# HybridRobotics/ilqr-iterative-tasks

Measured on AMD Instinct MI355X. Metric: batched iLQR iterations/s (n=6,m=2,N=20), higher is better.
Workload: dtype f64

## Files before the change

ilqr_iterative_tasks_amd/csrc/i2lqr_abi.hip:

```cpp
#include <hip/hip_runtime.h>
#include <dlfcn.h>
#include <rccl/rccl.h>

#include <atomic>
#include <cmath>
#include <cstdarg>
#include <cstdio>
#include <cstdlib>
#include <cstring>
#include <mutex>
#include <new>
#include <unordered_set>

#include "../../include/i2lqr.h"
#include "i2lqr_devcfg.hpp"
#include "i2lqr_geometry.hpp"
#include "i2lqr_group.h"
#include "i2lqr_lane.hpp"
#include "i2lqr_select.hpp"
#include "i2lqr_wave.hpp"

#include "i2lqr_lane12.h"

#define I2LQR_DRY_RUN_LANE 1
// ... 233 lines not shown
}

struct i2lqr_handle {
  i2lqr_config cfg;
  int lanes;
  size_t lds_bytes;
  int device;
  void* ws;
  int64_t ws_bytes;
  int64_t compact_min_batch;
  int opt_defer, opt_reroll, opt_lds_steps, opt_merge, opt_ckpt, opt_stagger;
  int wave_tail;
  int opt_pair;
  int opt_two_x;
  int opt_chunk_step;
  int opt_fuse;
  int opt_final_round;
  int opt_first_chunk;
  int opt_fstep;
  int opt_group;
  int opt_spec;
  int opt_group_ws;
  int opt_group_overlap;
  struct Epilogue {
    const int32_t* qfun;
    int outer_iter, max_relax_iter;
    void* cost_it;
    void* part;
    int64_t* best_idx;
    void* best_cost;
    bool fused;
  };
  static constexpr unsigned kTickets = 16;
  unsigned* ticket;
  std::atomic<unsigned> ticket_next;
  hipEvent_t ev_ready, ev_side_done;
  bool side_pending;
  DeviceGeometry geo;
};

namespace {
thread_local i2lqr_handle::Epilogue* t_epi = nullptr;
}

namespace {

// ... 142 lines not shown
        a.best_idx = t_epi->best_idx;
        a.best_cost = (T*)t_epi->best_cost;
      }
      t_epi->fused = true;
    }
    switch (fk) {
      case K_INVALID:
        return fail(I2LQR_ERR_UNSUPPORTED, "%s", why);
      case K_SPEC:
      case K_SPEC16:
        if constexpr (m == 2 && n + m <= 8) {
          HIP_TRY(group_spec_iterate<T>(h->cfg, a, s, fk == K_SPEC16 ? 16 : 8));
          return I2LQR_OK;
        }
        break;
      case K_GROUP:
        if constexpr (m == 2 && n + m <= 8) {
          HIP_TRY(group_iterate<T>(h->cfg, a, s));
          return I2LQR_OK;
        }
        break;
      case K_GROUP16:
        if constexpr (m == 2 && n + m <= 8) {
          HIP_TRY(group16_iterate<T>(h->cfg, a, s, h->opt_group_overlap != 0));
          return I2LQR_OK;
        }
        break;
      case K_GROUP_WS:
        if constexpr (m == 2 && n + m <= 8) {
          HIP_TRY(group_iterate_ws<T>(h->cfg, a, h->ws, s));
          return I2LQR_OK;
        }
        break;
      case K_QUAD:
        if constexpr (n + m == 16) {
          HIP_TRY(quad_iterate<T>(h->cfg, a, h->ws, s));
          return I2LQR_OK;
        }
        break;
      case K_WAVE:
        break;
    }
    const size_t lds_f = fstep_lds_bytes(h->cfg.N);
    const int64_t waves_per_cu = (grid(B) + h->geo.cus - 1) / h->geo.cus;
    const bool fstep = kHasFstep && lds_f <= h->geo.default_dyn_lds &&
                       (h->opt_fstep >= 0 ? h->opt_fstep != 0
                                          : waves_per_cu * lds_f <= h->geo.lds_per_cu - 10 * 1024);
// ... 812 lines not shown
#ifdef I2LQR_DRY_RUN
  const bool dry_run = dry::on();
#else
  constexpr bool dry_run = false;
#endif
  if (!dry_run && (hipGetDeviceCount(&ndev) != hipSuccess || ndev <= 0))
    return fail(I2LQR_ERR_NODEVICE, "no HIP device visible (this library has no CPU path)");
  i2lqr_handle* h = new (std::nothrow) i2lqr_handle;
  if (!h) return fail(I2LQR_ERR_LAUNCH, "out of host memory");
  h->cfg = *cfg;
  h->geo = device_geometry();
  if (h->geo.wave != 64) {
    const int w = h->geo.wave;
    delete h;
    return fail(I2LQR_ERR_UNSUPPORTED, "the kernels are built for 64-lane wavefronts (gfx950), this "
                "device reports %d", w);
  }
  h->ws = nullptr;
  h->ws_bytes = 0;
  h->compact_min_batch = -1;
  h->opt_defer = h->opt_reroll = h->opt_lds_steps = h->opt_fstep = h->opt_group = -1;
  h->opt_merge = h->opt_ckpt = h->opt_spec = h->opt_stagger = h->opt_group_ws = -1;
  h->opt_group_overlap = -1;
  h->wave_tail = -1;
  h->opt_first_chunk = -1;
  h->opt_fuse = -1;
  h->opt_final_round = -1;
  h->opt_chunk_step = -1;
  h->opt_pair = -1;
  h->opt_two_x = -1;
  h->ticket = nullptr;
  h->ticket_next.store(0);
  h->ev_ready = h->ev_side_done = nullptr;
  h->side_pending = false;
  constexpr size_t kTicketBytes = i2lqr_handle::kTickets * sizeof(unsigned);
  if (dry_run) {
#ifdef I2LQR_DRY_RUN
    static unsigned fake_tickets[i2lqr_handle::kTickets];
    h->device = 0;
    h->ticket = fake_tickets;
    dry::allow(fake_tickets, sizeof(fake_tickets));
#endif
  } else if (hipGetDevice(&h->device) != hipSuccess ||
      hipMalloc((void**)&h->ticket, kTicketBytes) != hipSuccess ||
      hipMemset(h->ticket, 0, kTicketBytes) != hipSuccess) {
    if (h->ticket) (void)hipFree(h->ticket);
// ... 152 lines not shown
}

int i2lqr_set_option(i2lqr_handle* h, const char* name, int64_t value) {
  if (!h || !name) return fail(I2LQR_ERR_INVALID, "null handle or option name");
  if (value < -1 || value > 0x7fffffff) return fail(I2LQR_ERR_INVALID, "option value out of range");
  const int v = (int)value;
  if (!strcmp(name, "defer_states")) h->opt_defer = v < 0 ? -1 : (v != 0);
  else if (!strcmp(name, "reroll_nominal")) h->opt_reroll = v < 0 ? -1 : (v != 0);
  else if (!strcmp(name, "lds_gain_steps")) h->opt_lds_steps = v;
  else if (!strcmp(name, "merge_inputs")) h->opt_merge = v < 0 ? -1 : (v != 0);
  else if (!strcmp(name, "checkpoint_states")) h->opt_ckpt = v < 0 ? -1 : (v != 0);
  else if (!strcmp(name, "stagger")) h->opt_stagger = v;
  else if (!strcmp(name, "per_step_jacobians")) h->opt_fstep = v < 0 ? -1 : (v != 0);
  else if (!strcmp(name, "wave_tail")) h->wave_tail = v < 0 ? -1 : (v > 65536 ? 65536 : v);
  else if (!strcmp(name, "first_chunk")) h->opt_first_chunk = v < 1 ? -1 : (v > 1024 ? 1024 : v);
  else if (!strcmp(name, "helper_wavefront")) h->opt_pair = v < 0 ? -1 : (v != 0);
  else if (!strcmp(name, "state_buffers")) h->opt_two_x = v < 0 ? -1 : (v != 0);
  else if (!strcmp(name, "chunk_step")) h->opt_chunk_step = v < 1 ? -1 : (v > 1024 ? 1024 : v);
  else if (!strcmp(name, "fused_compaction")) h->opt_fuse = v < 0 ? -1 : (v != 0);
  else if (!strcmp(name, "final_round")) h->opt_final_round = v < 0 ? -1 : (v > 20 ? 20 : v);
  else if (!strcmp(name, "speculate")) h->opt_spec = v < 0 ? -1 : (v != 0);
  else if (!strcmp(name, "group_workspace")) h->opt_group_ws = v < 0 ? -1 : (v != 0);
  else if (!strcmp(name, "group_overlap")) h->opt_group_overlap = v < 0 ? -1 : (v != 0);
  else if (!strcmp(name, "debug_self_test")) {
#ifdef I2LQR_DEBUG
    unsigned long long* w = i2lqr::debug_trap_word();
    double* buf = nullptr;
    HIP_TRY(hipMalloc((void**)&buf, 8 * sizeof(double)));
    hipLaunchKernelGGL(k_debug_self_test, dim3(1), dim3(64), 0, (hipStream_t)0, buf, w);
    const int rc = debug_check(I2LQR_OK, nullptr);
    (void)hipFree(buf);
    return rc;
#else
    return fail(I2LQR_ERR_UNSUPPORTED, "\"debug_self_test\" exists in the index-checked debug build "
                "only (make -C ilqr_iterative_tasks_amd/csrc debug)");
#endif
  }
  else if (!strcmp(name, "group_lanes")) {
    if (v != -1 && v != 8 && v != 16 && v != 64)
      return fail(I2LQR_ERR_INVALID, "\"group_lanes\" is 8, 16, 64 or -1");
    h->opt_group = v;
  }
  else return fail(I2LQR_ERR_INVALID, "unknown option '%s'", name);
  return I2LQR_OK;
}

// ... 588 lines not shown
```

ilqr_iterative_tasks_amd/csrc/i2lqr_group.h:

```cpp
#pragma once
#include <hip/hip_runtime.h>

#include "../../include/i2lqr.h"
#include "i2lqr_wave.hpp"

namespace i2lqr {

bool group_supported(const i2lqr_config& cfg);
template <class T> hipError_t group_iterate(const i2lqr_config& cfg, const IterArgs<T>& a,
                                            hipStream_t stream);

constexpr int64_t kGroup16Batch = 4096;
bool group16_supported(const i2lqr_config& cfg);
template <class T> hipError_t group16_iterate(const i2lqr_config& cfg, const IterArgs<T>& a,
                                              hipStream_t stream, bool overlap = true);

constexpr int64_t kGroupWsBatch = 4096;
constexpr int64_t kGroupWsTop = 8192;
constexpr int64_t kGroupWsTopF32 = 7168;
inline int64_t group_ws_top(const i2lqr_config& cfg) {
  return cfg.dtype == I2LQR_F64 ? kGroupWsTop : kGroupWsTopF32;
}
int64_t group_workspace_bytes(const i2lqr_config& cfg, int64_t B);
template <class T> hipError_t group_iterate_ws(const i2lqr_config& cfg, const IterArgs<T>& a,
                                               void* ws, hipStream_t stream);

bool group_spec_supported(const i2lqr_config& cfg, int lanes);
template <class T> hipError_t group_spec_iterate(const i2lqr_config& cfg, const IterArgs<T>& a,
                                                 hipStream_t stream, int lanes);
bool group_spec_chain_supported(const i2lqr_config& cfg, int64_t chains);
template <class T> hipError_t group_spec_chain(const i2lqr_config& cfg, const IterArgs<T>& a,
                                               hipStream_t stream);
bool group_spec_tail_supported(const i2lqr_config& cfg);
template <class T> hipError_t group_spec_tail(const i2lqr_config& cfg, const IterArgs<T>& a,
                                              hipStream_t stream);

bool quad_supported(const i2lqr_config& cfg);
int64_t quad_workspace_bytes(const i2lqr_config& cfg, int64_t B);
// ... 5 lines not shown
```

ilqr_iterative_tasks_amd/csrc/i2lqr_group.hip:

```cpp
#include "i2lqr_group.h"

#include "i2lqr_devcfg.hpp"
#include "i2lqr_geometry.hpp"
#include "i2lqr_group.hpp"
#include "i2lqr_dryrun.hpp"

namespace i2lqr {

namespace {

template <class T, class Sys, int G = kGroup> size_t group_lds_bytes(int N) {
  return (size_t)GLayout<Sys, G>(N).wave_words() * sizeof(T);
}

template <auto Kernel> hipError_t raise_lds_limit(size_t lds) {
  if (lds <= device_geometry().default_dyn_lds) return hipSuccess;
  constexpr int kMaxDev = 64;
  static thread_local int raised_for[kMaxDev] = {};
  int dev = 0;
  hipError_t e = hipGetDevice(&dev);
  if (e != hipSuccess) return e;
  if (dev < 0 || dev >= kMaxDev || raised_for[dev] < (int)lds) {
    e = hipFuncSetAttribute((const void*)Kernel, hipFuncAttributeMaxDynamicSharedMemorySize,
                            (int)lds);
    if (e != hipSuccess) return e;
    if (dev >= 0 && dev < kMaxDev) raised_for[dev] = (int)lds;
  }
  return hipSuccess;
}

template <class T, class Sys, int H, int G = kGroup>
hipError_t launch_h(const i2lqr_config& cfg, const IterArgs<T>& a, hipStream_t s) {
  const auto c = make_dev_cfg<T, Sys::n, Sys::m>(cfg);
  const size_t lds = group_lds_bytes<T, Sys, G>(cfg.N);
  if (hipError_t e = raise_lds_limit<k_group_iterate<T, Sys, H, false, G>>(lds); e != hipSuccess)
    return e;
  constexpr int PW = 64 / G;
  const unsigned grid = (unsigned)((a.B + PW - 1) / PW);
  hipLaunchKernelGGL((k_group_iterate<T, Sys, H, false, G>), dim3(grid), dim3(64 * H), lds, s, c, a,
                     (T*)nullptr);
  return hipGetLastError();
}
template <class T, class Sys>
hipError_t launch16(const i2lqr_config& cfg, const IterArgs<T>& a, hipStream_t s, bool overlap) {
  const int64_t cus = device_geometry().cus;
#ifndef I2LQR_STAMPS
  if (overlap && (a.B + 3) / 4 <= cus) return launch_h<T, Sys, 3, 16>(cfg, a, s);
  if ((a.B + 3) / 4 <= 2 * cus) return launch_h<T, Sys, 2, 16>(cfg, a, s);
#endif
  return launch_h<T, Sys, 1, 16>(cfg, a, s);
}
template <class T, class Sys>
hipError_t launch_ws(const i2lqr_config& cfg, const IterArgs<T>& a, void* ws, hipStream_t s) {
  const auto c = make_dev_cfg<T, Sys::n, Sys::m>(cfg);
  const size_t lds = (size_t)GLayout<Sys>(cfg.N, true).wave_words() * sizeof(T);
  if (hipError_t e = raise_lds_limit<k_group_iterate<T, Sys, 1, true>>(lds); e != hipSuccess) return e;
  const unsigned grid = (unsigned)((a.B + kGroupsPerWave - 1) / kGroupsPerWave);
  hipLaunchKernelGGL((k_group_iterate<T, Sys, 1, true>), dim3(grid), dim3(64), lds, s, c, a, (T*)ws);
  return hipGetLastError();
}

template <class T, class Sys>
hipError_t launch(const i2lqr_config& cfg, const IterArgs<T>& a, hipStream_t s) {
  const int64_t cus = device_geometry().cus;
#ifndef I2LQR_STAMPS
  if ((a.B + kGroupsPerWave - 1) / kGroupsPerWave <= cus) return launch_h<T, Sys, 3>(cfg, a, s);
#endif
  return launch_h<T, Sys, 1>(cfg, a, s);
}

constexpr int kSpecWideBatch = 512;

// ... 76 lines not shown
  if (chains > geo.scaled(kSpecWideBatch)) return false;
  const size_t lds = visit_bicycle(cfg, [&](auto t, auto sys) {
    return spec_lds_bytes<decltype(t), decltype(sys), 3, 16>(cfg.N);
  });
  return lds <= geo.max_dyn_lds;
}
template <class T>
hipError_t group_spec_chain(const i2lqr_config& cfg, const IterArgs<T>& a, hipStream_t s) {
  return visit_bicycle<T>(cfg, [&](auto, auto sys) {
    return launch_spec_chain<T, decltype(sys)>(cfg, a, s);
  });
}
template <class T>
hipError_t group_spec_iterate(const i2lqr_config& cfg, const IterArgs<T>& a, hipStream_t s, int lanes) {
  return launch_spec_any<T, false>(cfg, a, s, lanes);
}
template <class T>
hipError_t group_spec_tail(const i2lqr_config& cfg, const IterArgs<T>& a, hipStream_t s) {
  return launch_spec_any<T, true>(cfg, a, s, group_spec_tail_lanes(cfg));
}

bool group16_supported(const i2lqr_config& cfg) { return group_lds_fits<16>(cfg); }
template <class T>
hipError_t group16_iterate(const i2lqr_config& cfg, const IterArgs<T>& a, hipStream_t s, bool overlap) {
  return visit_bicycle<T>(cfg, [&](auto, auto sys) {
    return launch16<T, decltype(sys)>(cfg, a, s, overlap);
  });
}

bool group_supported(const i2lqr_config& cfg) { return group_lds_fits<kGroup>(cfg); }

int64_t group_workspace_bytes(const i2lqr_config& cfg, int64_t B) {
  if (!group_supported(cfg) || B <= 0) return 0;
  const int64_t probs = (B + kGroupsPerWave - 1) / kGroupsPerWave * kGroupsPerWave;
  const int64_t words = visit_bicycle<double>(cfg, [&](auto, auto sys) {
    return GLayout<decltype(sys)>(cfg.N, true).ws_words();
  });
  const size_t lds = visit_bicycle(cfg, [&](auto t, auto sys) {
    return (size_t)GLayout<decltype(sys)>(cfg.N, true).wave_words() * sizeof(t);
  });
  if (lds > device_geometry().max_dyn_lds) return 0;
  return probs * words * (cfg.dtype == I2LQR_F64 ? 8 : 4);
}
template <class T>
hipError_t group_iterate_ws(const i2lqr_config& cfg, const IterArgs<T>& a, void* ws, hipStream_t s) {
  return visit_bicycle<T>(cfg, [&](auto, auto sys) {
    return launch_ws<T, decltype(sys)>(cfg, a, ws, s);
  });
}

template <class T>
hipError_t group_iterate(const i2lqr_config& cfg, const IterArgs<T>& a, hipStream_t s) {
  return visit_bicycle<T>(cfg, [&](auto, auto sys) { return launch<T, decltype(sys)>(cfg, a, s); });
}

#define I2LQR_GROUP_LAUNCHERS(T)                                                                    \
  template hipError_t group_iterate<T>(const i2lqr_config&, const IterArgs<T>&, hipStream_t);       \
  template hipError_t group16_iterate<T>(const i2lqr_config&, const IterArgs<T>&, hipStream_t, bool); \
  template hipError_t group_iterate_ws<T>(const i2lqr_config&, const IterArgs<T>&, void*,           \
                                          hipStream_t);                                             \
  template hipError_t group_spec_iterate<T>(const i2lqr_config&, const IterArgs<T>&, hipStream_t,   \
                                            int);                                                   \
  template hipError_t group_spec_chain<T>(const i2lqr_config&, const IterArgs<T>&, hipStream_t);    \
  template hipError_t group_spec_tail<T>(const i2lqr_config&, const IterArgs<T>&, hipStream_t);
I2LQR_GROUP_LAUNCHERS(double)
I2LQR_GROUP_LAUNCHERS(float)

}
```

ilqr_iterative_tasks_amd/csrc/i2lqr_group.hpp:

```cpp
#pragma once
#include <hip/hip_runtime.h>
#include <stdint.h>

#include "i2lqr_systems.hpp"
#include "i2lqr_wave.hpp"

namespace i2lqr {

constexpr int kGroup = 8;
constexpr int kGroupsPerWave = 64 / kGroup;

template <class Sys> struct GroupPattern {
  static constexpr int n = Sys::n, m = Sys::m, W = n + m, NV = Sys::NVAR;
  static constexpr int dt_row(int b) {
    for (int i = 2; i < n; i++)
      if (i != b && Sys::pat(i, b) == 2) return i;
    return -1;
  }
  static constexpr bool column_ok(int b) {
    int extra = 0;
    for (int i = 0; i < n; i++) {
      const int code = Sys::pat(i, b);
      if (i < 2) {
        if (code == 2) return false;
// ... 61 lines not shown
template <int L, class T, int R>
__device__ __forceinline__ void bcast_fmac(T (&a)[R], const T (&s)[R], T c) {
#pragma unroll
  for (int r = 0; r < R; r++) bcast_fmac1<L>(a[r], s[r], c);
}
template <int L> __device__ __forceinline__ double bcast_mov(double v) {
  long long x = __builtin_bit_cast(long long, v);
  x = __builtin_amdgcn_mov_dpp(x, 0x150 + L, 0xf, 0xf, false);
  return __builtin_bit_cast(double, x);
}
template <int L> __device__ __forceinline__ float bcast_mov(float v) {
  int x = __builtin_bit_cast(int, v);
  x = __builtin_amdgcn_mov_dpp(x, 0x150 + L, 0xf, 0xf, false);
  return __builtin_bit_cast(float, x);
}
template <class T, int R> __device__ __forceinline__ void dpp_ready(T (&v)[R]) {
  if constexpr (R == 8)
    asm("s_nop 1" : "+v"(v[0]), "+v"(v[1]), "+v"(v[2]), "+v"(v[3]), "+v"(v[4]), "+v"(v[5]), "+v"(v[6]), "+v"(v[7]));
  else if constexpr (R == 6)
    asm("s_nop 1" : "+v"(v[0]), "+v"(v[1]), "+v"(v[2]), "+v"(v[3]), "+v"(v[4]), "+v"(v[5]));
  else static_assert(R == 6 || R == 8, "dpp_ready: n + m of the bicycles");
}

template <class T, class Sys, bool WS = false, int G = kGroup> struct GroupWorker {
  static constexpr int n = Sys::n, m = Sys::m, W = n + m, NV = Sys::NVAR, NT = Sys::NTRIG;
  static constexpr int NA = n + 1;
  using Cfg = DevCfg<T, n, m>;
  using GL = GLayout<Sys, G>;
  static_assert(G == kGroup || G == 16, "eight lanes per problem, or one 16-lane DPP row");
  static_assert(G == kGroup || !WS, "the workspace form is built for eight lanes per problem");
  using GP = GroupPattern<Sys>;
  static_assert(GP::ok(), "plant does not have the column structure this kernel is written for");
  const Cfg& c;
  const GL L;
  const Slice<T> S;
  const T* const Qt;
  const int g;
  const int N;
  int oR, oKk;
  T* T1c;
  int rho;
  T* Wp = nullptr;

  int off_c0, off_c1;
  int off_l0, off_l1;
  int off_lu[m];
  T own, cdt;
  int rsrc;
#ifdef I2LQR_STAMPS
  mutable unsigned long long st_acc[8] = {0, 0, 0, 0, 0, 0, 0, 0}, st_t0 = 0, st_t1 = 0;
#endif

  __device__ GroupWorker(const Cfg& c_, T* smem, int lane)
      : GroupWorker(c_, smem + (lane / G) * GL(c_.N, WS).total,
                    smem + GL(c_.N, WS).qt_base(), lane % G,
                    GL(c_.N, WS).total) {
    const int p = lane / G;
    if constexpr (G == kGroup) T1c = smem + L.t1_base() + p * GL::kT1Stride;
    rho = (p >> 1) & 1;
  }
  __device__ __forceinline__ T* rec(int t) const {
    if constexpr (WS) return Wp + L.ws_rec() + t * GL::RW;
    else return S + oR + t * GL::RW;
  }
  __device__ __forceinline__ T* gain(int t) const {
    if constexpr (WS) return Wp + L.ws_gain() + t * (m * GL::KW);
    else return S + oKk + t * (m * GL::KW);
  }
  __device__ __forceinline__ T* gain_x(int t) const {
    if constexpr (WS) return S + oKk;
    else return S + oKk + t * (m * GL::KW);
  }
  __device__ __forceinline__ void ws_publish() const {
    if constexpr (WS) {
      __builtin_amdgcn_fence(__ATOMIC_RELEASE, "workgroup");
      __builtin_amdgcn_s_waitcnt(0);
      wave_sync();
      __builtin_amdgcn_fence(__ATOMIC_ACQUIRE, "workgroup");
    }
  }
  __device__ __forceinline__ int t1_word(int col, int row) const {
    return (row >> 1) * (2 * kGroup) + ((col + rho) & (kGroup - 1)) * 2 + (row & 1);
  }

  __device__ GroupWorker(const Cfg& c_, T* slice, const T* qt, int g_, int slice_words)
      : c(c_), L(c_.N, WS), S(make_slice(slice, slice_words, c_.trap, TAG_GROUP_LDS)), Qt(qt),
        g(g_), N(c_.N) {
    oR = L.R; oKk = L.Kk;
    T1c = nullptr;
    rho = 0;
    off_c0 = GL::R_ZERO; off_c1 = GL::R_ZERO; off_l0 = GL::R_ZERO; off_l1 = GL::R_ZERO;
#pragma unroll
    for (int a = 0; a < m; a++) off_lu[a] = GL::R_ZERO;
    own = T(0); cdt = T(0); rsrc = 0;
    static_for_i<0, W>([&](auto b_) {
      constexpr int b = decltype(b_)::value;
      if (g == b && b < n) {
        constexpr int c0 = Sys::pat(0, b), c1 = Sys::pat(1, b);
        off_c0 = c0 == 0 ? GL::R_ZERO : (c0 == 1 ? GL::R_ONE : GL::R_JV + (c0 - 3));
        off_c1 = c1 == 0 ? GL::R_ZERO : (c1 == 1 ? GL::R_ONE : GL::R_JV + (c1 - 3));
        own = (b >= 2) ? T(1) : T(0);
        constexpr int r = GP::dt_row(b);
        cdt = r >= 0 ? c.dt : T(0);
        rsrc = r >= 0 ? r : 0;
        if (b < 2) {
          off_l0 = GL::R_OB + 2 + b;
          off_l1 = GL::R_OB + 3 + b;
        }
      }
    });
// ... 25 lines not shown
    }
    return acc;
  }

  template <int i, int a> __device__ __forceinline__ void f_acc(T& acc, bool& first, T v,
                                                                const T (&jv)[NV]) const {
    constexpr int code = Sys::pat(i, a);
    if constexpr (code == 0) {
      return;
    } else if constexpr (code == 1) {
      acc = first ? v : acc + v;
      first = false;
    } else {
      const T f = code == 2 ? c.dt : jv[code >= 3 ? code - 3 : 0];
      acc = first ? f * v : t_fma(f, v, acc);
      first = false;
    }
  }

  __device__ __forceinline__ T rollout(int XUo, int TRo, const T (&xT)[n]) const {
    T x[n], u[m], xn[n], tr[NT];
#pragma unroll
    for (int i = 0; i < n; i++) x[i] = S[XUo + i];
    for (int t = 0; t < N; t++) {
#pragma unroll
      for (int a = 0; a < m; a++) u[a] = clip(S[XUo + t * W + n + a], -c.u_max[a], c.u_max[a]);
#pragma unroll
      for (int a = 0; a < m; a++) S[XUo + t * W + n + a] = u[a];
      Sys::trig(x, tr);
#pragma unroll
      for (int q = 0; q < NT; q++) S[TRo + t * NT + q] = tr[q];
      Sys::step_tr(c, x, u, tr, xn);
#pragma unroll
      for (int i = 0; i < n; i++) S[XUo + (t + 1) * W + i] = xn[i];
#pragma unroll
      for (int i = 0; i < n; i++) x[i] = xn[i];
    }
    Sys::trig(x, tr);
#pragma unroll
    for (int q = 0; q < NT; q++) S[TRo + N * NT + q] = tr[q];
    const T cost = terminal_cost(x, xT);
    wave_sync();
    return cost;
  }

  __device__ __forceinline__ void prep(int XUo, int TRo, const T (&ob)[6], T pa, T pb, int first,
// ... 243 lines not shown
      for (int r = 0; r < n; r++) vx += (T(2) * Qt[i * n + r]) * dx[r];
      const T vxx = T(2) * Qt[i * n + gq];
      vb[i] = (g == n) ? vx : (g < n ? vxx : T(0));
    }
  }
  template <bool GENERAL>
  __device__ __forceinline__ bool backward_row_from(const T (&vb)[n], T lamb, bool commit) const {
    static_assert(GL::KW > n + 1, "the padding word of a gain row takes the stores of idle lanes");
    bool bad = false;
    T va[n];
    {
      const T* Rn = rec(N);
#pragma unroll
      for (int i = 0; i < n; i++) va[i] = vb[i];
      va[0] += Rn[off_l0];
      va[1] += Rn[off_l1];
    }
    const int gcol = (commit && g <= n) ? g : GL::KW - 1;
    T cdr[n];
#pragma unroll
    for (int r = 0; r < n; r++) cdr[r] = (rsrc == r) ? cdt : T(0);
    struct Rec { T jv[NV], luu[m], c0, c1, l0, l1, lrow[m]; };
    Rec ra, rb;
    auto load_record = [&](int t, Rec& r) __attribute__((always_inline)) {
      const T* R = rec(t);
#pragma unroll
      for (int q = 0; q < NV; q++) r.jv[q] = R[GL::R_JV + q];
#pragma unroll
      for (int a = 0; a < m; a++) r.luu[a] = R[GL::R_LUU + a];
      r.c0 = R[off_c0];
      r.c1 = R[off_c1];
      r.l0 = R[off_l0];
      r.l1 = R[off_l1];
#pragma unroll
      for (int a = 0; a < m; a++) r.lrow[a] = R[off_lu[a]];
    };
    auto f_entry = [&](auto k_, auto b_, const T (&jv)[NV]) __attribute__((always_inline)) {
      constexpr int code = Sys::pat(decltype(k_)::value, n + decltype(b_)::value);
      if constexpr (code == 1) return T(1);
      else if constexpr (code == 2) return c.dt;
      else return jv[code >= 3 ? code - 3 : 0];
    };
    load_record(N - 1, ra);
    auto step = [&](const int t, Rec& rc, Rec& rn) __attribute__((always_inline)) {
      const T (&jv)[NV] = rc.jv;
      T t1[W];
      static_for_i<0, W>([&](auto a_) {
        constexpr int a = decltype(a_)::value;
        T acc = T(0);
        bool first = true;
        static_for_i<0, n>([&](auto i_) {
          constexpr int i = decltype(i_)::value;
          f_acc<i, a>(acc, first, va[i], jv);
        });
        t1[a] = acc;
      });
      dpp_ready(t1);
      load_record(t > 0 ? t - 1 : 0, rn);
// ... 54 lines not shown
      T* Kt = gain_x(t);
#pragma unroll
      for (int a = 0; a < m; a++) Kt[a * GL::KW + gcol] = kc[a];
      T qk[m];
#pragma unroll
      for (int a = 0; a < m; a++) {
        T acc = T(0);
#pragma unroll
        for (int b = 0; b < m; b++) acc = t_fma(Quu[a * m + b], kc[b], acc);
        qk[a] = acc;
      }
      T vn[n];
#pragma unroll
      for (int i = 0; i < n; i++) vn[i] = hx[i];
      static_for_i<0, n>([&](auto i_) {
        constexpr int i = decltype(i_)::value;
#pragma unroll
        for (int a = 0; a < m; a++) bcast_fmac1<i>(vn[i], pk[a], qk[a]);
      });
#pragma unroll
      for (int i = 0; i < n; i++) va[i] = vn[i];
    };
    STAMP_BEGIN();
    int t = N - 1;
    if constexpr (I2LQR_GROUP_UNROLL >= 4) {
      for (; t >= 3; t -= 4) {
        step(t, ra, rb);
        step(t - 1, rb, ra);
        step(t - 2, ra, rb);
        step(t - 3, rb, ra);
      }
    }
    for (; t >= 1; t -= 2) {
      step(t, ra, rb);
      step(t - 1, rb, ra);
    }
    if (t == 0) step(0, ra, rb);
    STAMP_END(1);
    wave_sync();
    return bad;
  }

  __device__ __forceinline__ T forward_row(int XUo, int XUn, int TRn, const T (&xT)[n],
                                           bool* bad) const {
    static_assert(G == 16 && m == 2, "two inputs on the two halves of a 16-lane row");
    const int half = g >> 3;
    const T umax = half ? c.u_max[1] : c.u_max[0];
    T x[n], u[m], xn[n], tr[NT];
#pragma unroll
    for (int i = 0; i < n; i++) x[i] = S[XUo + i];
#pragma unroll
    for (int i = 0; i < n; i++) S[XUn + i] = x[i];
    Sys::template trig_g<false>(x, tr, bad);
#pragma unroll
    for (int q = 0; q < NT; q++) S[TRn + q] = tr[q];
    static_assert(!WS, "gain rows and records are neighbours in the LDS slice");
    auto pXo = S + XUo;
    auto pXn = S + XUn;
    auto pG = S + (oKk + half * GL::KW);
    auto pTR = S + (TRn + half * NT);
// ... 3 lines not shown
#pragma unroll
      for (int j = 0; j < n; j++) xo[j] = pXo[k * W + j];
      uo = pXo[k * W + n + half];
#pragma unroll
      for (int j = 0; j < NA; j++) kk[j] = pG[k * (m * GL::KW) + j];
    };
    load_step(std::integral_constant<int, 0>{});
    auto step = [&](auto k_, const T (&trc)[NT]) __attribute__((always_inline)) {
      constexpr int k = decltype(k_)::value;
      T acc = T(0);
#pragma unroll
      for (int j = 0; j < n; j++) acc = t_fma(kk[j], x[j] - xo[j], acc);
      const T ua = clip(uo + kk[n] + acc, -umax, umax);
      load_step(std::integral_constant<int, k + 1>{});
      pXn[k * W + n + half] = ua;
      u[0] = bcast_mov<0>(ua);
      u[1] = bcast_mov<8>(ua);
      Sys::step_tr(c, x, u, trc, xn);
#pragma unroll
      for (int i = 0; i < n; i++) pXn[(k + 1) * W + i] = xn[i];
#pragma unroll
      for (int i = 0; i < n; i++) x[i] = xn[i];
    };
    int t = 0;
    for (; t + 1 < N; t += 2) {
      step(std::integral_constant<int, 0>{}, tr);
      T sc[NT], tr1[NT];
      Sys::trig_heading_fast(half ? Sys::next_heading(c, x) : Sys::heading(x), sc, bad);
#pragma unroll
      for (int q = 0; q < NT; q++) pTR[NT + q] = sc[q];
#pragma unroll
      for (int q = 0; q < NT; q++) {
        tr1[q] = bcast_mov<0>(sc[q]);
        tr[q] = bcast_mov<8>(sc[q]);
      }
      step(std::integral_constant<int, 1>{}, tr1);
      pXo = pXo + 2 * W;
      pXn = pXn + 2 * W;
      pG = pG + 2 * (m * GL::KW);
      pTR = pTR + 2 * NT;
    }
    if (t < N) {
      step(std::integral_constant<int, 0>{}, tr);
      Sys::template trig_g<false>(x, tr, bad);
#pragma unroll
      for (int q = 0; q < NT; q++) S[TRn + N * NT + q] = tr[q];
    }
    const T cost = terminal_cost(x, xT);
    wave_sync();
    return cost;
  }

  template <bool GENERAL>
  __device__ __forceinline__ T forward(int XUo, int XUn, int TRn, const T (&xT)[n],
                                       bool* bad) const {
    if constexpr (G == 16 && !GENERAL && Sys::kHeadingAhead && m == 2)
      return forward_row(XUo, XUn, TRn, xT, bad);
    T x[n], u[m], xn[n], tr[NT];
#pragma unroll
    for (int i = 0; i < n; i++) x[i] = S[XUo + i];
#pragma unroll
    for (int i = 0; i < n; i++) S[XUn + i] = x[i];
    T xo[n], uo[m];
    struct Gains { T kk[m][NA]; };
    Gains ga, gb;
    auto load_gains = [&](int t, Gains& q) __attribute__((always_inline)) {
      const T* Kg = gain(t);
#pragma unroll
      for (int a = 0; a < m; a++)
#pragma unroll
        for (int j = 0; j < NA; j++) q.kk[a][j] = Kg[a * GL::KW + j];
    };
    auto load_step = [&](int t, Gains& q) __attribute__((always_inline)) {
#pragma unroll
      for (int j = 0; j < n; j++) xo[j] = S[XUo + t * W + j];
#pragma unroll
      for (int a = 0; a < m; a++) uo[a] = S[XUo + t * W + n + a];
      if constexpr (!WS) load_gains(t, q);
    };
    if constexpr (WS) {
// ... 45 lines not shown
      for (; t + 1 < N; t += 2) {
        step(t, ga, ga);
        step(t + 1, ga, ga);
      }
      if (t < N) step(t, ga, ga);
    }
    Sys::template trig_g<GENERAL>(x, tr, bad);
#pragma unroll
    for (int q = 0; q < NT; q++) S[TRn + N * NT + q] = tr[q];
    const T cost = terminal_cost(x, xT);
    wave_sync();
    return cost;
  }
};

__device__ __forceinline__ int idx_div(int e, int d, float rcp_d) {
  int q = (int)((float)e * rcp_d);
  const int r = e - q * d;
  q += (r >= d) ? 1 : 0;
  q -= (r < 0) ? 1 : 0;
  return q;
}

template <class T, class Sys, int H = 1, bool WS = false, int G = kGroup>
__global__ __launch_bounds__(64 * H) void k_group_iterate(const DevCfg<T, Sys::n, Sys::m> c,
                                                          const IterArgs<T> a, T* ws = nullptr) {
  static_assert(!(WS && H > 1), "the workspace form runs without helper wavefronts");
  constexpr int n = Sys::n, m = Sys::m, W = n + m;
#ifdef I2LQR_STAMPS
  constexpr bool OVL = false;
#else
  constexpr bool OVL = G == 16 && H >= 3;
#endif
  using GL = GLayout<Sys, G>;
  extern __shared__ __align__(16) unsigned char gsmem_raw[];
  T* smem = reinterpret_cast<T*>(gsmem_raw);
  const int lane = threadIdx.x & 63, hv = threadIdx.x >> 6;
#ifdef I2LQR_STAMPS
  unsigned long long st_k0, st_k1, st_k2, st_k3;
  asm volatile("s_memtime %0\n\ts_waitcnt lgkmcnt(0)" : "=s"(st_k0)::"memory");
#endif
  const int64_t prob0 = (int64_t)blockIdx.x * GL::PW + lane / G;
  const bool real = prob0 < a.B;
  const int64_t prob = real ? prob0 : a.B - 1;
  GroupWorker<T, Sys, WS, G> w(c, smem, lane);
  const int N = c.N, g = w.g;
  const float rN = 1.0f / (float)N, rN1 = 1.0f / (float)(N + 1), rnN = 1.0f / (float)(n * N);
  const GL& L = w.L;
  const auto S = w.S;
  if constexpr (WS) w.Wp = ws + prob0 * (int64_t)L.ws_words();

  if (H == 1 || hv == 0) {
    const T* gX = a.X + prob * (int64_t)(n * (N + 1));
    if (g < n) S[L.XU0 + g] = gX[g * (N + 1)];
    const T* gU = a.U + prob * (int64_t)(m * N);
    for (int e = g; e < m * N; e += G) {
      const int aa = idx_div(e, N, rN), t = e - aa * N;
      S[L.XU0 + t * W + n + aa] = gU[e];
    }
    for (int e = lane; e < n * n; e += 64) smem[L.qt_base() + e] = c.Qt[e];
  }
  T xT[n], ob[6];
#pragma unroll
  for (int i = 0; i < n; i++) xT[i] = a.x_term[prob * n + i];
#pragma unroll
  for (int q = 0; q < 6; q++) ob[q] = a.obs ? a.obs[prob * 6 + q] : T(q == 5 ? -1 : 1);
  T lamb = a.lamb[prob];
  wave_sync();

// ... 180 lines not shown
    w.st_acc[2] = st_k1 - st_k0;
    w.st_acc[3] = st_k2 - st_k1;
    w.st_acc[4] = st_k3 - st_k2;
    if (a.dbg && g == 0)
      for (int q = 0; q < 8; q++) a.dbg[prob * 8 + q] = w.st_acc[q];
#endif
  }
  if (a.qfun) {
    const bool cand = real && g == 0;
    T ci = T(0);
    if (cand) {
      const int XUo = cur ? L.XU1 : L.XU0;
      double ss = 0.0;
#pragma unroll
      for (int i = 0; i < n; i++) {
        const double d = (double)S[XUo + N * W + i] - (double)xT[i];
        ss += d * d;
      }
      ci = (T)relax_cost_value(ss, a.qfun[prob], N, a.outer_iter, a.max_relax_iter);
      a.cost_it[prob] = ci;
    }
    if (a.pick_part) pick_epilogue(a, cand, prob, ci);
  }
}

template <class Sys, int V, int G = kGroup> struct GSpecLayout {
  static constexpr int n = Sys::n, m = Sys::m, W = n + m, NT = Sys::NTRIG;
  static constexpr int PW = 64 / G;
  using GL = GLayout<Sys, G>;
  int N;
  int traj_words, R, var0, var_words, Kk_in_var, T1c_in_var, total;
  __host__ __device__ explicit GSpecLayout(int N_) : N(N_) {
    const int xu = (W * (N + 1) + 3) & ~3, tr = (NT * (N + 1) + 3) & ~3;
    traj_words = xu + tr;
    int o = (V + 1) * traj_words;
    R = o; o += GL::RW * (N + 1); o = (o + 3) & ~3;
    var0 = o;
    Kk_in_var = 0;
    T1c_in_var = (m * GL::KW * N + 3) & ~3;
    var_words = G == kGroup ? (T1c_in_var + kGroup * 2 * ((W + 1) / 2) + 3) & ~3
                            : (T1c_in_var + m * GL::KW + 3) & ~3;
    o += V * var_words;
    if (((o / 4) & 1) == 0) o += 4;
    total = o;
  }
  __host__ __device__ int xu_off(int b) const { return b * traj_words; }
// ... 216 lines not shown
```

Before: 74.74 million.

## Add compile-time horizon specialization of the 16-lane group kernel for N=20

Adds a kernel instantiation in which the horizon N is a template constant (only 20 for now). With it the backward and forward sweeps unroll completely and the LDS record offsets become compile-time strides from fixed base pointers. This is meant to remove loop overhead and runtime address arithmetic from the per-step recursions. The fixed path is selected by default whenever N matches. In exchange it adds code size and register pressure, plus another kernel per helper-wavefront count.

```diff
diff --git a/ilqr_iterative_tasks_amd/csrc/i2lqr_abi.hip b/ilqr_iterative_tasks_amd/csrc/i2lqr_abi.hip
--- a/ilqr_iterative_tasks_amd/csrc/i2lqr_abi.hip
+++ b/ilqr_iterative_tasks_amd/csrc/i2lqr_abi.hip
@@ -279,6 +279,7 @@
   int opt_spec;
   int opt_group_ws;
   int opt_group_overlap;
+  int opt_group_fixed;
   struct Epilogue {
     const int32_t* qfun;
     int outer_iter, max_relax_iter;
@@ -467,7 +468,8 @@
         break;
       case K_GROUP16:
         if constexpr (m == 2 && n + m <= 8) {
-          HIP_TRY(group16_iterate<T>(h->cfg, a, s, h->opt_group_overlap != 0));
+          HIP_TRY(group16_iterate<T>(h->cfg, a, s, h->opt_group_overlap != 0,
+                                     h->opt_group_fixed != 0));
           return I2LQR_OK;
         }
         break;
@@ -1326,6 +1328,7 @@
   h->opt_defer = h->opt_reroll = h->opt_lds_steps = h->opt_fstep = h->opt_group = -1;
   h->opt_merge = h->opt_ckpt = h->opt_spec = h->opt_stagger = h->opt_group_ws = -1;
   h->opt_group_overlap = -1;
+  h->opt_group_fixed = -1;
   h->wave_tail = -1;
   h->opt_first_chunk = -1;
   h->opt_fuse = -1;
@@ -1524,6 +1527,7 @@
   else if (!strcmp(name, "speculate")) h->opt_spec = v < 0 ? -1 : (v != 0);
   else if (!strcmp(name, "group_workspace")) h->opt_group_ws = v < 0 ? -1 : (v != 0);
   else if (!strcmp(name, "group_overlap")) h->opt_group_overlap = v < 0 ? -1 : (v != 0);
+  else if (!strcmp(name, "group_fixed_horizon")) h->opt_group_fixed = v < 0 ? -1 : (v != 0);
   else if (!strcmp(name, "debug_self_test")) {
 #ifdef I2LQR_DEBUG
     unsigned long long* w = i2lqr::debug_trap_word();
diff --git a/ilqr_iterative_tasks_amd/csrc/i2lqr_group.h b/ilqr_iterative_tasks_amd/csrc/i2lqr_group.h
--- a/ilqr_iterative_tasks_amd/csrc/i2lqr_group.h
+++ b/ilqr_iterative_tasks_amd/csrc/i2lqr_group.h
@@ -13,7 +13,12 @@
 constexpr int64_t kGroup16Batch = 4096;
 bool group16_supported(const i2lqr_config& cfg);
 template <class T> hipError_t group16_iterate(const i2lqr_config& cfg, const IterArgs<T>& a,
-                                              hipStream_t stream, bool overlap = true);
+                                              hipStream_t stream, bool overlap = true,
+                                              bool fixed = true);
+#define I2LQR_GROUP_FIXED_HORIZONS(X) X(20)
+bool group16_fixed_horizon(int N);
+template <class T> hipError_t group16_iterate_fixed(const i2lqr_config& cfg, const IterArgs<T>& a,
+                                                    hipStream_t stream, int wavefronts);
 
 constexpr int64_t kGroupWsBatch = 4096;
 constexpr int64_t kGroupWsTop = 8192;
diff --git a/ilqr_iterative_tasks_amd/csrc/i2lqr_group.hip b/ilqr_iterative_tasks_amd/csrc/i2lqr_group.hip
--- a/ilqr_iterative_tasks_amd/csrc/i2lqr_group.hip
+++ b/ilqr_iterative_tasks_amd/csrc/i2lqr_group.hip
@@ -4,30 +4,11 @@
 #include "i2lqr_geometry.hpp"
 #include "i2lqr_group.hpp"
 #include "i2lqr_dryrun.hpp"
+#include "i2lqr_group_launch.hpp"
 
 namespace i2lqr {
 
 namespace {
-
-template <class T, class Sys, int G = kGroup> size_t group_lds_bytes(int N) {
-  return (size_t)GLayout<Sys, G>(N).wave_words() * sizeof(T);
-}
-
-template <auto Kernel> hipError_t raise_lds_limit(size_t lds) {
-  if (lds <= device_geometry().default_dyn_lds) return hipSuccess;
-  constexpr int kMaxDev = 64;
-  static thread_local int raised_for[kMaxDev] = {};
-  int dev = 0;
-  hipError_t e = hipGetDevice(&dev);
-  if (e != hipSuccess) return e;
-  if (dev < 0 || dev >= kMaxDev || raised_for[dev] < (int)lds) {
-    e = hipFuncSetAttribute((const void*)Kernel, hipFuncAttributeMaxDynamicSharedMemorySize,
-                            (int)lds);
-    if (e != hipSuccess) return e;
-    if (dev >= 0 && dev < kMaxDev) raised_for[dev] = (int)lds;
-  }
-  return hipSuccess;
-}
 
 template <class T, class Sys, int H, int G = kGroup>
 hipError_t launch_h(const i2lqr_config& cfg, const IterArgs<T>& a, hipStream_t s) {
@@ -42,12 +23,17 @@
   return hipGetLastError();
 }
 template <class T, class Sys>
-hipError_t launch16(const i2lqr_config& cfg, const IterArgs<T>& a, hipStream_t s, bool overlap) {
+hipError_t launch16(const i2lqr_config& cfg, const IterArgs<T>& a, hipStream_t s, bool overlap,
+                    bool fixed) {
   const int64_t cus = device_geometry().cus;
+  int wavefronts = 1;
 #ifndef I2LQR_STAMPS
-  if (overlap && (a.B + 3) / 4 <= cus) return launch_h<T, Sys, 3, 16>(cfg, a, s);
-  if ((a.B + 3) / 4 <= 2 * cus) return launch_h<T, Sys, 2, 16>(cfg, a, s);
+  if (overlap && (a.B + 3) / 4 <= cus) wavefronts = 3;
+  else if ((a.B + 3) / 4 <= 2 * cus) wavefronts = 2;
+  if (fixed && group16_fixed_horizon(cfg.N)) return group16_iterate_fixed<T>(cfg, a, s, wavefronts);
 #endif
+  if (wavefronts == 3) return launch_h<T, Sys, 3, 16>(cfg, a, s);
+  if (wavefronts == 2) return launch_h<T, Sys, 2, 16>(cfg, a, s);
   return launch_h<T, Sys, 1, 16>(cfg, a, s);
 }
 template <class T, class Sys>
@@ -170,9 +156,10 @@
 
 bool group16_supported(const i2lqr_config& cfg) { return group_lds_fits<16>(cfg); }
 template <class T>
-hipError_t group16_iterate(const i2lqr_config& cfg, const IterArgs<T>& a, hipStream_t s, bool overlap) {
-  return visit_bicycle<T>(cfg, [&](auto, auto sys) {
-    return launch16<T, decltype(sys)>(cfg, a, s, overlap);
+hipError_t group16_iterate(const i2lqr_config& cfg, const IterArgs<T>& a, hipStream_t s, bool overlap,
+                           bool fixed) {
+  return visit_bicycle<T>(cfg, [&](auto, auto sys) {
+    return launch16<T, decltype(sys)>(cfg, a, s, overlap, fixed);
   });
 }
 
@@ -204,7 +191,8 @@
 
 #define I2LQR_GROUP_LAUNCHERS(T)                                                                    \
   template hipError_t group_iterate<T>(const i2lqr_config&, const IterArgs<T>&, hipStream_t);       \
-  template hipError_t group16_iterate<T>(const i2lqr_config&, const IterArgs<T>&, hipStream_t, bool); \
+  template hipError_t group16_iterate<T>(const i2lqr_config&, const IterArgs<T>&, hipStream_t, bool, \
+                                         bool);                                                    \
   template hipError_t group_iterate_ws<T>(const i2lqr_config&, const IterArgs<T>&, void*,           \
                                           hipStream_t);                                             \
   template hipError_t group_spec_iterate<T>(const i2lqr_config&, const IterArgs<T>&, hipStream_t,   \
diff --git a/ilqr_iterative_tasks_amd/csrc/i2lqr_group.hpp b/ilqr_iterative_tasks_amd/csrc/i2lqr_group.hpp
--- a/ilqr_iterative_tasks_amd/csrc/i2lqr_group.hpp
+++ b/ilqr_iterative_tasks_amd/csrc/i2lqr_group.hpp
@@ -107,13 +107,15 @@
   else static_assert(R == 6 || R == 8, "dpp_ready: n + m of the bicycles");
 }
 
-template <class T, class Sys, bool WS = false, int G = kGroup> struct GroupWorker {
+template <class T, class Sys, bool WS = false, int G = kGroup, int NH = 0> struct GroupWorker {
   static constexpr int n = Sys::n, m = Sys::m, W = n + m, NV = Sys::NVAR, NT = Sys::NTRIG;
   static constexpr int NA = n + 1;
   using Cfg = DevCfg<T, n, m>;
   using GL = GLayout<Sys, G>;
   static_assert(G == kGroup || G == 16, "eight lanes per problem, or one 16-lane DPP row");
   static_assert(G == kGroup || !WS, "the workspace form is built for eight lanes per problem");
+  static_assert(NH == 0 || (G == 16 && !WS), "the fixed-horizon form is the sixteen-lane LDS form");
+  static __host__ __device__ constexpr int horizon(int cfg_N) { return NH > 0 ? NH : cfg_N; }
   using GP = GroupPattern<Sys>;
   static_assert(GP::ok(), "plant does not have the column structure this kernel is written for");
   const Cfg& c;
@@ -122,6 +124,10 @@
   const T* const Qt;
   const int g;
   const int N;
+  __device__ __forceinline__ int loop_N() const {
+    if constexpr (NH > 0) return c.N;
+    else return N;
+  }
   int oR, oKk;
   T* T1c;
   int rho;
@@ -137,9 +143,9 @@
 #endif
 
   __device__ GroupWorker(const Cfg& c_, T* smem, int lane)
-      : GroupWorker(c_, smem + (lane / G) * GL(c_.N, WS).total,
-                    smem + GL(c_.N, WS).qt_base(), lane % G,
-                    GL(c_.N, WS).total) {
+      : GroupWorker(c_, smem + (lane / G) * GL(horizon(c_.N), WS).total,
+                    smem + GL(horizon(c_.N), WS).qt_base(), lane % G,
+                    GL(horizon(c_.N), WS).total) {
     const int p = lane / G;
     if constexpr (G == kGroup) T1c = smem + L.t1_base() + p * GL::kT1Stride;
     rho = (p >> 1) & 1;
@@ -169,8 +175,8 @@
   }
 
   __device__ GroupWorker(const Cfg& c_, T* slice, const T* qt, int g_, int slice_words)
-      : c(c_), L(c_.N, WS), S(make_slice(slice, slice_words, c_.trap, TAG_GROUP_LDS)), Qt(qt),
-        g(g_), N(c_.N) {
+      : c(c_), L(horizon(c_.N), WS), S(make_slice(slice, slice_words, c_.trap, TAG_GROUP_LDS)),
+        Qt(qt), g(g_), N(horizon(c_.N)) {
     oR = L.R; oKk = L.Kk;
     T1c = nullptr;
     rho = 0;
@@ -242,6 +248,7 @@
     T x[n], u[m], xn[n], tr[NT];
 #pragma unroll
     for (int i = 0; i < n; i++) x[i] = S[XUo + i];
+    const int N = loop_N();
     for (int t = 0; t < N; t++) {
 #pragma unroll
       for (int a = 0; a < m; a++) u[a] = clip(S[XUo + t * W + n + a], -c.u_max[a], c.u_max[a]);
@@ -531,18 +538,42 @@
     for (int r = 0; r < n; r++) cdr[r] = (rsrc == r) ? cdt : T(0);
     struct Rec { T jv[NV], luu[m], c0, c1, l0, l1, lrow[m]; };
     Rec ra, rb;
+    constexpr bool FIXED = NH > 0 && !GENERAL;
+    const T* const R0 = rec(0);
+    const T *pc0 = R0, *pc1 = R0, *pl0 = R0, *pl1 = R0, *plu[m];
+#pragma unroll
+    for (int a = 0; a < m; a++) plu[a] = R0;
+    if constexpr (FIXED) {
+      pc0 = R0 + off_c0; pc1 = R0 + off_c1; pl0 = R0 + off_l0; pl1 = R0 + off_l1;
+#pragma unroll
+      for (int a = 0; a < m; a++) plu[a] = R0 + off_lu[a];
+    }
     auto load_record = [&](int t, Rec& r) __attribute__((always_inline)) {
-      const T* R = rec(t);
-#pragma unroll
-      for (int q = 0; q < NV; q++) r.jv[q] = R[GL::R_JV + q];
-#pragma unroll
-      for (int a = 0; a < m; a++) r.luu[a] = R[GL::R_LUU + a];
-      r.c0 = R[off_c0];
-      r.c1 = R[off_c1];
-      r.l0 = R[off_l0];
-      r.l1 = R[off_l1];
-#pragma unroll
-      for (int a = 0; a < m; a++) r.lrow[a] = R[off_lu[a]];
+      if constexpr (FIXED) {
+        const int o = t * GL::RW;
+#pragma unroll
+        for (int q = 0; q < NV; q++) r.jv[q] = R0[o + GL::R_JV + q];
+#pragma unroll
+        for (int a = 0; a < m; a++) r.luu[a] = R0[o + GL::R_LUU + a];
+        r.c0 = pc0[o];
+        r.c1 = pc1[o];
+        r.l0 = pl0[o];
+        r.l1 = pl1[o];
+#pragma unroll
+        for (int a = 0; a < m; a++) r.lrow[a] = plu[a][o];
+      } else {
+        const T* R = rec(t);
+#pragma unroll
+        for (int q = 0; q < NV; q++) r.jv[q] = R[GL::R_JV + q];
+#pragma unroll
+        for (int a = 0; a < m; a++) r.luu[a] = R[GL::R_LUU + a];
+        r.c0 = R[off_c0];
+        r.c1 = R[off_c1];
+        r.l0 = R[off_l0];
+        r.l1 = R[off_l1];
+#pragma unroll
+        for (int a = 0; a < m; a++) r.lrow[a] = R[off_lu[a]];
+      }
     };
     auto f_entry = [&](auto k_, auto b_, const T (&jv)[NV]) __attribute__((always_inline)) {
       constexpr int code = Sys::pat(decltype(k_)::value, n + decltype(b_)::value);
@@ -643,20 +674,28 @@
       for (int i = 0; i < n; i++) va[i] = vn[i];
     };
     STAMP_BEGIN();
-    int t = N - 1;
-    if constexpr (I2LQR_GROUP_UNROLL >= 4) {
-      for (; t >= 3; t -= 4) {
+    if constexpr (FIXED) {
+      static_for_i<0, NH>([&](auto i_) {
+        constexpr int i = decltype(i_)::value;
+        if constexpr (i % 2 == 0) step(NH - 1 - i, ra, rb);
+        else step(NH - 1 - i, rb, ra);
+      });
+    } else {
+      int t = loop_N() - 1;
+      if constexpr (I2LQR_GROUP_UNROLL >= 4) {
+        for (; t >= 3; t -= 4) {
+          step(t, ra, rb);
+          step(t - 1, rb, ra);
+          step(t - 2, ra, rb);
+          step(t - 3, rb, ra);
+        }
+      }
+      for (; t >= 1; t -= 2) {
         step(t, ra, rb);
         step(t - 1, rb, ra);
-        step(t - 2, ra, rb);
-        step(t - 3, rb, ra);
-      }
-    }
-    for (; t >= 1; t -= 2) {
-      step(t, ra, rb);
-      step(t - 1, rb, ra);
-    }
-    if (t == 0) step(0, ra, rb);
+      }
+      if (t == 0) step(0, ra, rb);
+    }
     STAMP_END(1);
     wave_sync();
     return bad;
@@ -706,30 +745,38 @@
 #pragma unroll
       for (int i = 0; i < n; i++) x[i] = xn[i];
     };
-    int t = 0;
-    for (; t + 1 < N; t += 2) {
-      step(std::integral_constant<int, 0>{}, tr);
-      T sc[NT], tr1[NT];
-      Sys::trig_heading_fast(half ? Sys::next_heading(c, x) : Sys::heading(x), sc, bad);
-#pragma unroll
-      for (int q = 0; q < NT; q++) pTR[NT + q] = sc[q];
-#pragma unroll
-      for (int q = 0; q < NT; q++) {
-        tr1[q] = bcast_mov<0>(sc[q]);
-        tr[q] = bcast_mov<8>(sc[q]);
-      }
-      step(std::integral_constant<int, 1>{}, tr1);
-      pXo = pXo + 2 * W;
-      pXn = pXn + 2 * W;
-      pG = pG + 2 * (m * GL::KW);
-      pTR = pTR + 2 * NT;
-    }
-    if (t < N) {
-      step(std::integral_constant<int, 0>{}, tr);
-      Sys::template trig_g<false>(x, tr, bad);
-#pragma unroll
-      for (int q = 0; q < NT; q++) S[TRn + N * NT + q] = tr[q];
-    }
+#define I2LQR_FORWARD_ROW_PAIR()                                                                   \
+    {                                                                                              \
+      step(std::integral_constant<int, 0>{}, tr);                                 \
+      T sc[NT], tr1[NT];                                                                           \
+      Sys::trig_heading_fast(half ? Sys::next_heading(c, x) : Sys::heading(x), sc, bad);           \
+      _Pragma("unroll") for (int q = 0; q < NT; q++) pTR[NT + q] = sc[q];  \
+      _Pragma("unroll") for (int q = 0; q < NT; q++) {                                             \
+        tr1[q] = bcast_mov<0>(sc[q]);                                                              \
+        tr[q] = bcast_mov<8>(sc[q]);                   \
+      }                                                                                            \
+      step(std::integral_constant<int, 1>{}, tr1);                                \
+      pXo = pXo + 2 * W;                                                                           \
+      pXn = pXn + 2 * W;                                                                           \
+      pG = pG + 2 * (m * GL::KW);                                                                  \
+      pTR = pTR + 2 * NT;                                                                          \
+    }
+#define I2LQR_FORWARD_ROW_LAST()                     \
+    {                                                                                              \
+      step(std::integral_constant<int, 0>{}, tr);                                                  \
+      Sys::template trig_g<false>(x, tr, bad);                                                     \
+      _Pragma("unroll") for (int q = 0; q < NT; q++) S[TRn + N * NT + q] = tr[q];                  \
+    }
+    if constexpr (NH > 0) {
+      static_for_i<0, NH / 2>([&](auto) __attribute__((always_inline)) I2LQR_FORWARD_ROW_PAIR());
+      if constexpr (NH % 2 != 0) I2LQR_FORWARD_ROW_LAST()
+    } else {
+      int t = 0;
+      for (; t + 1 < N; t += 2) I2LQR_FORWARD_ROW_PAIR()
+      if (t < N) I2LQR_FORWARD_ROW_LAST()
+    }
+#undef I2LQR_FORWARD_ROW_PAIR
+#undef I2LQR_FORWARD_ROW_LAST
     const T cost = terminal_cost(x, xT);
     wave_sync();
     return cost;
@@ -740,6 +787,7 @@
                                        bool* bad) const {
     if constexpr (G == 16 && !GENERAL && Sys::kHeadingAhead && m == 2)
       return forward_row(XUo, XUn, TRn, xT, bad);
+    const int N = loop_N();
     T x[n], u[m], xn[n], tr[NT];
 #pragma unroll
     for (int i = 0; i < n; i++) x[i] = S[XUo + i];
@@ -831,9 +879,9 @@
   return q;
 }
 
-template <class T, class Sys, int H = 1, bool WS = false, int G = kGroup>
-__global__ __launch_bounds__(64 * H) void k_group_iterate(const DevCfg<T, Sys::n, Sys::m> c,
-                                                          const IterArgs<T> a, T* ws = nullptr) {
+template <class T, class Sys, int H, bool WS, int G, int NH>
+__device__ __forceinline__ void group_iterate_body(const DevCfg<T, Sys::n, Sys::m>& c,
+                                                   const IterArgs<T>& a, T* ws) {
   static_assert(!(WS && H > 1), "the workspace form runs without helper wavefronts");
   constexpr int n = Sys::n, m = Sys::m, W = n + m;
 #ifdef I2LQR_STAMPS
@@ -852,8 +900,8 @@
   const int64_t prob0 = (int64_t)blockIdx.x * GL::PW + lane / G;
   const bool real = prob0 < a.B;
   const int64_t prob = real ? prob0 : a.B - 1;
-  GroupWorker<T, Sys, WS, G> w(c, smem, lane);
-  const int N = c.N, g = w.g;
+  GroupWorker<T, Sys, WS, G, NH> w(c, smem, lane);
+  const int N = NH > 0 ? NH : c.N, g = w.g;
   const float rN = 1.0f / (float)N, rN1 = 1.0f / (float)(N + 1), rnN = 1.0f / (float)(n * N);
   const GL& L = w.L;
   const auto S = w.S;
@@ -1080,6 +1128,19 @@
     }
     if (a.pick_part) pick_epilogue(a, cand, prob, ci);
   }
+}
+
+template <class T, class Sys, int H = 1, bool WS = false, int G = kGroup>
+__global__ __launch_bounds__(64 * H) void k_group_iterate(const DevCfg<T, Sys::n, Sys::m> c,
+                                                          const IterArgs<T> a, T* ws = nullptr) {
+  group_iterate_body<T, Sys, H, WS, G, 0>(c, a, ws);
+}
+
+template <class T, class Sys, int H, int NH>
+__global__ __launch_bounds__(64 * H) void k_group_iterate_fixed(const DevCfg<T, Sys::n, Sys::m> c,
+                                                                const IterArgs<T> a) {
+  static_assert(NH > 0, "a compile-time horizon");
+  group_iterate_body<T, Sys, H, false, 16, NH>(c, a, nullptr);
 }
 
 template <class Sys, int V, int G = kGroup> struct GSpecLayout {
diff --git a/ilqr_iterative_tasks_amd/csrc/i2lqr_group_fixed.hip b/ilqr_iterative_tasks_amd/csrc/i2lqr_group_fixed.hip
--- /dev/null
+++ b/ilqr_iterative_tasks_amd/csrc/i2lqr_group_fixed.hip
@@ -0,0 +1,55 @@
+#include "i2lqr_group.h"
+
+#include "i2lqr_devcfg.hpp"
+#include "i2lqr_group.hpp"
+#include "i2lqr_dryrun.hpp"
+#include "i2lqr_group_launch.hpp"
+
+namespace i2lqr {
+
+namespace {
+
+template <class T, class Sys, int H, int NH>
+hipError_t launch_fixed_h(const i2lqr_config& cfg, const IterArgs<T>& a, hipStream_t s) {
+  const auto c = make_dev_cfg<T, Sys::n, Sys::m>(cfg);
+  const size_t lds = group_lds_bytes<T, Sys, 16>(cfg.N);
+  if (hipError_t e = raise_lds_limit<k_group_iterate_fixed<T, Sys, H, NH>>(lds); e != hipSuccess)
+    return e;
+  const unsigned grid = (unsigned)((a.B + 3) / 4);
+  hipLaunchKernelGGL((k_group_iterate_fixed<T, Sys, H, NH>), dim3(grid), dim3(64 * H), lds, s, c, a);
+  return hipGetLastError();
+}
+template <class T, class Sys, int NH>
+hipError_t launch_fixed(const i2lqr_config& cfg, const IterArgs<T>& a, hipStream_t s, int helpers) {
+  if (helpers == 3) return launch_fixed_h<T, Sys, 3, NH>(cfg, a, s);
+  if (helpers == 2) return launch_fixed_h<T, Sys, 2, NH>(cfg, a, s);
+  return launch_fixed_h<T, Sys, 1, NH>(cfg, a, s);
+}
+
+}
+
+bool group16_fixed_horizon(int N) {
+#define I2LQR_X(NH) if (N == NH) return true;
+  I2LQR_GROUP_FIXED_HORIZONS(I2LQR_X)
+#undef I2LQR_X
+  return false;
+}
+
+template <class T>
+hipError_t group16_iterate_fixed(const i2lqr_config& cfg, const IterArgs<T>& a, hipStream_t s,
+                                 int wavefronts) {
+  return visit_bicycle<T>(cfg, [&](auto, auto sys) -> hipError_t {
+    using Sys = decltype(sys);
+#define I2LQR_X(NH) if (cfg.N == NH) return launch_fixed<T, Sys, NH>(cfg, a, s, wavefronts);
+    I2LQR_GROUP_FIXED_HORIZONS(I2LQR_X)
+#undef I2LQR_X
+    return hipErrorInvalidValue;
+  });
+}
+
+template hipError_t group16_iterate_fixed<double>(const i2lqr_config&, const IterArgs<double>&,
+                                                  hipStream_t, int);
+template hipError_t group16_iterate_fixed<float>(const i2lqr_config&, const IterArgs<float>&,
+                                                 hipStream_t, int);
+
+}
diff --git a/ilqr_iterative_tasks_amd/csrc/i2lqr_group_launch.hpp b/ilqr_iterative_tasks_amd/csrc/i2lqr_group_launch.hpp
--- /dev/null
+++ b/ilqr_iterative_tasks_amd/csrc/i2lqr_group_launch.hpp
@@ -0,0 +1,29 @@
+#pragma once
+#include <hip/hip_runtime.h>
+
+#include "i2lqr_geometry.hpp"
+#include "i2lqr_group.hpp"
+
+namespace i2lqr {
+
+template <class T, class Sys, int G = kGroup> size_t group_lds_bytes(int N) {
+  return (size_t)GLayout<Sys, G>(N).wave_words() * sizeof(T);
+}
+
+template <auto Kernel> hipError_t raise_lds_limit(size_t lds) {
+  if (lds <= device_geometry().default_dyn_lds) return hipSuccess;
+  constexpr int kMaxDev = 64;
+  static thread_local int raised_for[kMaxDev] = {};
+  int dev = 0;
+  hipError_t e = hipGetDevice(&dev);
+  if (e != hipSuccess) return e;
+  if (dev < 0 || dev >= kMaxDev || raised_for[dev] < (int)lds) {
+    e = hipFuncSetAttribute((const void*)Kernel, hipFuncAttributeMaxDynamicSharedMemorySize,
+                            (int)lds);
+    if (e != hipSuccess) return e;
+    if (dev >= 0 && dev < kMaxDev) raised_for[dev] = (int)lds;
+  }
+  return hipSuccess;
+}
+
+}
```

Result: faster. 81.98 million (median of 6 runs) (+9.7%).
